# JiLiBIT/LIO-SLAM

Hardware: AMD Instinct MI355X
Metric: scan-to-map registrations/sec, 64x1800 scan vs 200-keyframe map; pose RMSE (higher is better)
Workload: dtype f32

## Files before the change

### include/liogpu.h

```cpp
#ifndef LIOGPU_H
#define LIOGPU_H

#include <stddef.h>
#include <stdint.h>

#ifdef __cplusplus
extern "C" {
#endif

#define LIO_VERSION 102
#define LIO_MAX_ITERS 32

enum {
    LIO_OK               = 0,
    LIO_TOO_FEW_POINTS   = 1,
    LIO_TOO_FEW_CORR     = 2,
    LIO_ERR_ARG          = -1,
    LIO_ERR_HIP          = -2,
    LIO_ERR_CAPACITY     = -3,
    LIO_ERR_NO_MAP       = -4,
    LIO_ERR_NO_DEVICE    = -5
};

typedef struct lio_s2m_config {
// ... 109 lines not shown
                                 float *coeff4, int32_t *nn_idx5);

int  lio_s2m_set_corner_map(lio_s2m_handle *h, const void *pts, size_t n, size_t stride_bytes);
int  lio_s2m_batch_upload_corners(lio_s2m_handle *h, int32_t n_scans, const void *const *scans,
                                  const size_t *n_pts, size_t stride_bytes);
int  lio_s2m_register_cs(lio_s2m_handle *h, const void *corner_scan, size_t n_corner,
                         const void *surf_scan, size_t n_surf, size_t stride_bytes,
                         float pose[6], lio_s2m_result *res);
int  lio_s2m_get_corner_correspondences(lio_s2m_handle *h, int32_t scan, uint8_t *flag,
                                        float *coeff4, int32_t *nn_idx5);

int  lio_s2m_get_profile(lio_s2m_handle *h, lio_s2m_profile *out);
int  lio_s2m_debug_persist_spin(lio_s2m_handle *h, int32_t spin_max, int32_t withhold_wg);

int  lio_debug_plane_fit(int32_t device_id, const float *sets, size_t n, double plane_tol, uint32_t *out);
int  lio_s2m_debug_stamps(lio_s2m_handle *h, long long *out, size_t cap_entries);

int  lio_s2m_set_stream(lio_s2m_handle *h, void *hip_stream);
int  lio_s2m_set_global_grid(lio_s2m_handle *h, const float origin[3], const int32_t dims[3]);
int  lio_s2m_set_shard(lio_s2m_handle *h, int32_t axis, int32_t lo, int32_t hi);
int  lio_s2m_set_shard_plan(lio_s2m_handle *h, int32_t axis, int32_t n_ranks, int32_t rank, const int32_t *bounds,
                            int32_t halo_cells);
int  lio_s2m_set_scan_shard(lio_s2m_handle *h, int32_t rank, int32_t world);
int  lio_s2m_batch_begin(lio_s2m_handle *h);
int  lio_s2m_batch_iter_partial(lio_s2m_handle *h, double *d_sums );
int  lio_s2m_batch_iter_apply(lio_s2m_handle *h, const double *d_sums);
int  lio_s2m_batch_n_active(lio_s2m_handle *h, int32_t *n_active);
int  lio_s2m_batch_poll_active(lio_s2m_handle *h, int32_t iteration, int32_t *n_active);

void lio_transform_update(float pose[6], int32_t imu_available, int32_t imu_type,
// ... 311 lines not shown
```

### lio-slam_amd/__init__.py

```python
from .api import (LioError, ScanToMap, S2MConfig, S2MResult, S2MProfile, DeskewConfig,
                  lib_path, load_library, build_library, deskew, curvature, imu_deskew_info,
                  transform_update, pack_xyzirt, deskew_default_config, voxel_grid, assemble_map, KeyframeStore, STATUS_NAMES,
                  extract_features, FeatureConfig, range_image, RangeImageConfig, PinnedBuffer, DeviceBuffer, PC2Layout, deskew_pc2,
                  NearbyConfig, nearby_default_config, IcpConfig, IcpResult, IcpClouds, ICP_STATES, icp_default_config, icp_align,
                  icp_debug_trace, ScConfig, ScResult, sc_default_config, sc_make, sc_distance,
                  LocalMapConfig, LocalMapInfo, sor_filter, local_map_default_config,
                  HeightMapConfig, HeightMapInfo, height_map, height_map_default_config,
                  GlobalMapConfig, GlobalMapInfo, ExportConfig, global_map_default_config, STAGED_DS, STAGED_RAW)

__all__ = ["LioError", "ScanToMap", "S2MConfig", "S2MResult", "S2MProfile", "DeskewConfig",
           "lib_path", "load_library", "build_library", "deskew", "curvature", "imu_deskew_info",
           "transform_update", "pack_xyzirt", "deskew_default_config", "voxel_grid", "assemble_map", "KeyframeStore", "STATUS_NAMES",
           "extract_features", "FeatureConfig", "range_image", "RangeImageConfig", "PinnedBuffer", "DeviceBuffer", "PC2Layout", "deskew_pc2",
           "NearbyConfig", "nearby_default_config", "IcpConfig", "IcpResult", "IcpClouds", "ICP_STATES", "icp_default_config", "icp_align",
           "icp_debug_trace", "ScConfig", "ScResult", "sc_default_config", "sc_make", "sc_distance",
           "LocalMapConfig", "LocalMapInfo", "sor_filter", "local_map_default_config",
           "HeightMapConfig", "HeightMapInfo", "height_map", "height_map_default_config",
           "GlobalMapConfig", "GlobalMapInfo", "ExportConfig", "global_map_default_config", "STAGED_DS", "STAGED_RAW"]
```

### lio-slam_amd/api.py

```python
import ctypes as C
import os
import subprocess

import numpy as np

_HERE = os.path.dirname(os.path.abspath(__file__))
LIO_MAX_ITERS = 32
STATUS_NAMES = {0: "OK", 1: "TOO_FEW_POINTS", 2: "TOO_FEW_CORR", -1: "ERR_ARG", -2: "ERR_HIP",
                -3: "ERR_CAPACITY", -4: "ERR_NO_MAP", -5: "ERR_NO_DEVICE"}


class LioError(RuntimeError):
    pass


class S2MConfig(C.Structure):
    _fields_ = [
        ("k", C.c_int32), ("max_sq_dist", C.c_float),
        ("plane_tol", C.c_double), ("weight", C.c_double), ("min_s", C.c_double),
        ("min_corr", C.c_int32), ("max_iters", C.c_int32), ("eig_thresh", C.c_float),
        ("conv_deg", C.c_double), ("conv_cm", C.c_double),
        ("min_scan_pts", C.c_int32), ("jacobian_mode", C.c_int32), ("force_all_iters", C.c_int32),
        ("device_id", C.c_int32), ("cell_size", C.c_float), ("max_batch", C.c_int32),
        ("max_scan_pts", C.c_int32), ("record_corr_iter", C.c_int32), ("kernel_variant", C.c_int32),
# ... 166 lines not shown
    "lio_curvature", "lio_s2m_debug_stamps", "lio_s2m_batch_poll_active", "lio_voxel_grid", "lio_assemble_map", "lio_kf_store_create", "lio_kf_store_destroy", "lio_kf_store_add",
    "lio_kf_store_count", "lio_kf_store_points", "lio_assemble_map_resident", "lio_s2m_set_scan_shard",
    "lio_s2m_set_corner_map", "lio_s2m_batch_upload_corners", "lio_s2m_register_cs",
    "lio_s2m_get_corner_correspondences", "lio_feature_default_config", "lio_extract_features",
    "lio_range_image_default_config", "lio_range_image",
    "lio_s2m_share_map", "lio_s2m_batch_upload_async", "lio_host_alloc", "lio_host_free", "lio_host_register",
    "lio_host_unregister", "lio_s2m_set_shard_plan", "lio_s2m_register_pc2", "lio_deskew_pc2", "lio_kf_store_add_device", "lio_kf_store_add_from_handle",
    "lio_s2m_register_raw", "lio_s2m_debug_persist_spin", "lio_device_alloc", "lio_device_free", "lio_device_upload",
    "lio_nearby_default_config", "lio_kf_store_set_poses", "lio_assemble_map_nearby", "lio_debug_plane_fit",
    "lio_icp_default_config", "lio_icp_align", "lio_kf_store_loop_icp", "lio_kf_store_detect_loop", "lio_icp_debug_trace",
    "lio_sc_default_config", "lio_sc_make", "lio_sc_distance", "lio_kf_store_sc_add", "lio_kf_store_sc_add_device",
    "lio_kf_store_sc_add_from_handle", "lio_kf_store_sc_count", "lio_kf_store_sc_geometry", "lio_kf_store_sc_get", "lio_kf_store_sc_detect",
    "lio_sor_filter", "lio_local_map_default_config", "lio_kf_store_local_map",
    "lio_height_map_default_config", "lio_height_map", "lio_kf_store_height_map",
    "lio_global_map_default_config", "lio_kf_store_global_map", "lio_kf_store_export_map", "lio_kf_store_get_keyframe",
    "lio_s2m_registered_cloud",
]


def load_library():
    global _LIB
    if _LIB is not None:
        return _LIB
    p = lib_path()
    if not os.path.exists(p):
        raise LioError(f"{p} is missing: run __graft_entry__.build() (hipcc --offload-arch=gfx950). "
                       "There is no CPU fallback.")
    L = C.CDLL(p)
    vp, i32, f32, f64, sz = C.c_void_p, C.c_int32, C.c_float, C.c_double, C.c_size_t
    L.lio_version.restype = C.c_int
    L.lio_last_error.restype = C.c_char_p
# ... 481 lines not shown
    for k, v in kw.items():
        setattr(c, k, v)
    return c


def curvature(rng, device_id=0):
    r = np.ascontiguousarray(rng, np.float32)
    curv = np.zeros(len(r), np.float32)
    picked = np.full(len(r), -1, np.int32)
    label = np.full(len(r), -1, np.int32)
    _check(load_library().lio_curvature(device_id, r.ctypes.data, len(r), curv.ctypes.data,
                                        picked.ctypes.data, label.ctypes.data), "lio_curvature")
    return curv, picked, label


def debug_plane_fit(sets, plane_tol=0.2, device_id=0):
    a = np.ascontiguousarray(sets, np.float32).reshape(-1, 15)
    out = np.zeros((len(a), 8), np.uint32)
    fn = load_library().lio_debug_plane_fit
    fn.argtypes = [C.c_int32, C.c_void_p, C.c_size_t, C.c_double, C.c_void_p]
    _check(fn(device_id, a.ctypes.data, len(a), float(plane_tol), out.ctypes.data), "lio_debug_plane_fit")
    return out


def range_image(records, t_cur, imu, device_id=0, **cfg_overrides):
    L = load_library()
    cfg = RangeImageConfig()
    L.lio_range_image_default_config(C.byref(cfg))
    cfg.device_id = device_id
    for k, v in cfg_overrides.items():
# ... 453 lines not shown
```

### lio-slam_amd/csrc/lio_device_math.h

```cpp
#pragma once
#include <hip/hip_runtime.h>
#include <float.h>
#include <stdint.h>

#define LIO_DEV __device__ __forceinline__

#ifndef LIO_SHARED_DIV
#define LIO_SHARED_DIV 1
#endif
struct LioDivisor { float d, r; bool mid; };

LIO_DEV bool lio_div_mid(float lo, float hi) { return lo >= 0x1p-40f && hi < 0x1p40f; }

LIO_DEV LioDivisor lio_divisor(float d)
{
    LioDivisor v;
    const float r0 = __builtin_amdgcn_rcpf(d);
    const float e = __builtin_fmaf(-d, r0, 1.0f);
    v.d = d; v.r = __builtin_fmaf(e, r0, r0);
    v.mid = lio_div_mid(fabsf(d), fabsf(d));
    return v;
}

LIO_DEV float lio_div_fast(float n, const LioDivisor& v)
// ... 147 lines not shown
            if (c[i] != 0.0f) {
                c[i] /= a[i][i];
#pragma unroll
                for (int r = 0; r < i; ++r) c[r] -= c[i] * a[r][i];
            }
        }
    }
    const float v0 = (0 < nz) ? c[0] : 0.0f;
    const float v1 = (1 < nz) ? c[1] : 0.0f;
    const float v2 = (2 < nz) ? c[2] : 0.0f;
#pragma unroll
    for (int j = 0; j < 3; ++j)
        x[j] = (p0 == j) ? v0 : (p1 == j) ? v1 : (p2 == j) ? v2 : 0.0f;
}

LIO_DEV bool lio_plane_fit5(const float m[5][3], double plane_tol, float X0[3], float& pa, float& pb, float& pc, float& pd)
{
    float a[5][3];
#pragma unroll
    for (int j = 0; j < 5; ++j) { a[j][0] = m[j][0]; a[j][1] = m[j][1]; a[j][2] = m[j][2]; }
    lio_plane_qr5x3(a, X0);
    pa = X0[0]; pb = X0[1]; pc = X0[2]; pd = 1;
    const float ps = sqrtf(pa * pa + pb * pb + pc * pc);
    const LioDivisor dv = lio_divisor(ps);
    if (LIO_SHARED_DIV && dv.mid && lio_div_mid(lio_min3_abs(pa, pb, pc), lio_max3_abs(pa, pb, pc))) {
        pa = lio_div_fast(pa, dv); pb = lio_div_fast(pb, dv); pc = lio_div_fast(pc, dv); pd = lio_div_fast(pd, dv);
    } else {
        pa /= ps; pb /= ps; pc /= ps; pd /= ps;
    }
    bool planeValid = true;
#pragma unroll
    for (int j = 0; j < 5; ++j) {
        const float v = fabsf(pa * m[j][0] + pb * m[j][1] + pc * m[j][2] + pd);
        if ((double)v > plane_tol) planeValid = false;
    }
    return planeValid;
}

LIO_DEV void lio_jacobian_row(const float tr[6], float px, float py, float pz,
                              float cx, float cy, float cz, float cw, int jac_exact,
                              float row[6], float &rhs)
{
    const float srx = tr[0], crx = tr[1], sry = tr[2], cry = tr[3], srz = tr[4], crz = tr[5];
    const float arx = (-srx * cry * px - (srx * sry * srz + crx * crz) * py + (crx * srz - srx * sry * crz) * pz) * cx
                    + (crx * cry * px - (srx * crz - crx * sry * srz) * py + (crx * sry * crz + srx * srz) * pz) * cy;
    const float mid = jac_exact ? (srx * cry * srz * py) : (srx * sry * srz * py);
    const float ary = (-crx * sry * px + crx * cry * srz * py + crx * cry * crz * pz) * cx
                    + (-srx * sry * px + mid + srx * cry * crz * pz) * cy
                    + (-cry * px - sry * srz * py - sry * crz * pz) * cz;
    const float arz = ((crx * sry * crz + srx * srz) * py + (srx * crz - crx * sry * srz) * pz) * cx
                    + ((-crx * srz + srx * sry * crz) * py + (-srx * sry * srz - crx * crz) * pz) * cy
                    + (cry * crz * py - cry * srz * pz) * cz;
    row[0] = arz; row[1] = ary; row[2] = arx;
    row[3] = cx;  row[4] = cy;  row[5] = cz;
    rhs = -cw;
}

__device__ static float lio_cv_hypot(float a, float b)
{
    a = fabsf(a); b = fabsf(b);
    if (a > b) { b /= a; return a * sqrtf(1 + b * b); }
    if (b > 0) { a /= b; return b * sqrtf(1 + a * a); }
    return 0.0f;
}

LIO_DEV void lio_eigen3_sym(float a00, float a01, float a02, float a11, float a12, float a22,
                            float& e0, float& e1, float axis[3])
// ... 41 lines not shown
#undef LIO_ROT
    }
    int m = 0;
    if (w0 < w1) m = 1;
    if ((m == 0 ? w0 : w1) < w2) m = 2;
    float t0;
#define LIO_SWAP(x, y) do { t0 = (x); (x) = (y); (y) = t0; } while (0)
    if (m == 1) { LIO_SWAP(w0, w1); LIO_SWAP(v00, v10); LIO_SWAP(v01, v11); LIO_SWAP(v02, v12); }
    if (m == 2) { LIO_SWAP(w0, w2); LIO_SWAP(v00, v20); LIO_SWAP(v01, v21); LIO_SWAP(v02, v22); }
    if (w1 < w2) LIO_SWAP(w1, w2);
#undef LIO_SWAP
    e0 = w0; e1 = w1;
    axis[0] = v00; axis[1] = v01; axis[2] = v02;
}

LIO_DEV bool lio_corner_assoc(const float m[5][3], float x0, float y0, float z0, double weight, double min_s,
                              float& ox, float& oy, float& oz, float& ow)
{
    float cx = 0, cy = 0, cz = 0;
#pragma unroll
    for (int j = 0; j < 5; ++j) { cx += m[j][0]; cy += m[j][1]; cz += m[j][2]; }
    cx /= 5; cy /= 5; cz /= 5;
    float a11 = 0, a12 = 0, a13 = 0, a22 = 0, a23 = 0, a33 = 0;
#pragma unroll
    for (int j = 0; j < 5; ++j) {
        const float ax = m[j][0] - cx, ay = m[j][1] - cy, az = m[j][2] - cz;
        a11 += ax * ax; a12 += ax * ay; a13 += ax * az;
        a22 += ay * ay; a23 += ay * az;
        a33 += az * az;
    }
    a11 /= 5; a12 /= 5; a13 /= 5; a22 /= 5; a23 /= 5; a33 /= 5;
// ... 4 lines not shown
    const float x1 = (float)((double)cx + 0.1 * (double)v[0]), y1 = (float)((double)cy + 0.1 * (double)v[1]),
                z1 = (float)((double)cz + 0.1 * (double)v[2]);
    const float x2 = (float)((double)cx - 0.1 * (double)v[0]), y2 = (float)((double)cy - 0.1 * (double)v[1]),
                z2 = (float)((double)cz - 0.1 * (double)v[2]);
    const float m1 = (x0 - x1) * (y0 - y2) - (x0 - x2) * (y0 - y1);
    const float m2 = (x0 - x1) * (z0 - z2) - (x0 - x2) * (z0 - z1);
    const float m3 = (y0 - y1) * (z0 - z2) - (y0 - y2) * (z0 - z1);
    const float a012 = sqrtf(m1 * m1 + m2 * m2 + m3 * m3);
    const float l12 = sqrtf((x1 - x2) * (x1 - x2) + (y1 - y2) * (y1 - y2) + (z1 - z2) * (z1 - z2));
    const float la = ((y1 - y2) * m1 + (z1 - z2) * m2) / a012 / l12;
    const float lb = -((x1 - x2) * m1 - (z1 - z2) * m3) / a012 / l12;
    const float lc = -((x1 - x2) * m2 + (y1 - y2) * m3) / a012 / l12;
    const float ld2 = a012 / l12;
    const float s = (float)(1 - weight * (double)fabsf(ld2));
    ox = s * la; oy = s * lb; oz = s * lc; ow = s * ld2;
    return (double)s > min_s;
}

struct LioSolveWs {
    float A[36];
    float B[36];
    float V2[36];
    float AtA[36];
    float X[6], X2[6];
};

__device__ static __forceinline__ int lio_solve6_qr_reg(float (&A)[36], float (&b)[6])
{
    const float eps = FLT_EPSILON * 10;
    float vl[6], hf[6];
#pragma unroll
// ... 254 lines not shown
```

### lio-slam_amd/csrc/lio_kernels.h

```cpp
#pragma once
#include <hip/hip_runtime.h>
#include "lio_types.h"

struct LioIterParams {
    LioGrid grid;
    LioShard shard;
    LioConsts c;
    const float4* map_sorted;
    const float4* map_xyz4;
    const int* cell_start;
    const float4* nbr_pts;
    const int* nbr_start;
    const float* sx;
    const float* sy;
    const float* sz;
    const int* perm;
    LioScanState* state;
    const LioBlockDesc* blocks;
    double* partials;
    unsigned* arrive;
    int max_blk;
    int xcd_remap;
    int* n_active;
    double* sums_out;
// ... 27 lines not shown
                           int n_blocks, unsigned char* skip, hipStream_t s);
void lio_launch_block_boxes(const LioBlockDesc* blocks, int n_blocks, const LioScanState* st, const float* sx, const float* sy,
                            const float* sz, float* box, hipStream_t s);
void lio_launch_scan_sort_lds(const void* stage, size_t stride, const LioScanState* st, int n_scans, int max_pts, float tile0,
                              int shard_axis, int* perm, float* x, float* y, float* z, hipStream_t s);
void lio_launch_scan_bbox(const void* stage, size_t stride, const LioBlockDesc* prep_blocks, int n_prep_blocks,
                          const LioScanState* st, unsigned* bbox, hipStream_t s);
void lio_launch_scan_tile_sort(const void* stage, size_t stride, int total_pts,
                               const LioBlockDesc* prep_blocks, int n_prep_blocks,
                               const LioScanState* st, const LioScanTiles* tiles, int n_keys,
                               int* key_of, int* key_count, int* key_start, int* tile_sums,
                               int* tmp_idx, int* perm, int* big_list, int* big_cnt,
                               float* x, float* y, float* z, hipStream_t s);
void lio_launch_exclusive_scan(const int* in, int n, int* tile_sums, int* out, hipStream_t s);
void lio_launch_xyzi4_to_soa(const float4* src, int n, float* x, float* y, float* z, float4* xyz4, hipStream_t s);
void lio_launch_debug_plane_fit(const float* sets, long long n, double plane_tol, unsigned* out, hipStream_t s);
```

### lio-slam_amd/csrc/lio_kernels.hip

```cpp
#include <hip/hip_runtime.h>
#include "lio_types.h"
#include "lio_device_math.h"
#include "lio_kernels.h"

#include "lio_s2m_device.h"
#include "lio_scan2.h"
#include "lio_wg.h"

__global__ void k_aos_to_soa(const unsigned char* __restrict__ src, size_t stride, int n,
                             float* __restrict__ x, float* __restrict__ y, float* __restrict__ z,
                             float4* __restrict__ xyz4 )
{
    int i = blockIdx.x * blockDim.x + threadIdx.x;
    if (i >= n) return;
    const float* p = reinterpret_cast<const float*>(src + (size_t)i * stride);
    const float a = p[0], b = p[1], c = p[2];
    x[i] = a; y[i] = b; z[i] = c;
    if (xyz4) xyz4[i] = make_float4(a, b, c, 0.0f);
}

__global__ void k_xyzi4_to_soa(const float4* __restrict__ src, int n, float* __restrict__ x, float* __restrict__ y,
                               float* __restrict__ z, float4* __restrict__ xyz4)
{
    const int i = blockIdx.x * blockDim.x + threadIdx.x;
// ... 550 lines not shown

template <bool SINGLE>
__global__ void k_s2m_init_state(LioScanState* __restrict__ st, int n_scans,
                                 float* __restrict__ poses, int from_state, LioConsts c, int* __restrict__ n_active)
{
    const int s = blockIdx.x * blockDim.x + threadIdx.x;
    bool enough = false;
    if (s < n_scans) {
        LioScanState* p = &st[s];
        float T[12], trig[6], pose[6];
        if (from_state) { for (int k = 0; k < 6; ++k) { pose[k] = p->pose[k]; poses[s * 6 + k] = pose[k]; } }
        else { for (int k = 0; k < 6; ++k) { pose[k] = poses[s * 6 + k]; p->pose[k] = pose[k]; } }
        lio_pose_to_transform(pose, T, trig);
        for (int k = 0; k < 12; ++k) p->T[k] = T[k];
        for (int k = 0; k < 6; ++k) p->trig[k] = trig[k];
        p->iter = 0; p->converged = 0; p->n_corr_last = 0;
        for (int k = 0; k < 32; ++k) { p->n_corr_iter[k] = 0; for (int j = 0; j < 6; ++j) p->pose_iter[k][j] = 0.0f; }
        for (int k = 0; k < 36; ++k) p->AtA[k] = 0.0f;
        for (int k = 0; k < 6; ++k) p->AtB[k] = 0.0f;
        enough = p->n_pts > c.min_scan_pts;
        p->done = enough ? 0 : 1;
        p->status = enough ? 0 : 1;
    }
    if (SINGLE) {
        const int n = __syncthreads_count(enough ? 1 : 0);
        if (threadIdx.x == 0) *n_active = n;
    } else if (enough) {
        atomicAdd(n_active, 1);
    }
}
// ... 229 lines not shown

        if (P.d5_cache && inr[pp])
            P.d5_cache[ci] = ok ? d2_5 : -1.0f;
        float cxx = 0.0f, cyy = 0.0f, czz = 0.0f, cww = 0.0f;
        bool accept = false;
        if (ok) accept = lio_assoc_point<CORNER>(P, nn, qx[pp], qy[pp], qz[pp], px[pp], py[pp], pz[pp], cxx, cyy, czz, cww);
        if (record && inr[pp]) {
            const int li = bd.first + pp * LIO_BLOCK + (int)threadIdx.x;
            const int oi = P.perm ? P.perm[base + li] : base + li;
            P.rec_flag[oi] = accept ? 1 : 0;
            reinterpret_cast<float4*>(P.rec_coeff)[oi] = make_float4(cxx, cyy, czz, cww);
#pragma unroll
            for (int j = 0; j < 5; ++j) P.rec_nn[(size_t)oi * 5 + j] = ok ? nn[j] : -1;
        }
        float row[6] = { 0.0f, 0.0f, 0.0f, 0.0f, 0.0f, 0.0f }, rhs = 0.0f;
        if (accept) lio_jacobian_row(tr, px[pp], py[pp], pz[pp], cxx, cyy, czz, cww, P.c.jac_exact, row, rhs);
        if (PPT > 1) __syncthreads();
        {
            double2* dst = reinterpret_cast<double2*>(s_rows[threadIdx.x]);
            dst[0] = make_double2((double)row[0], (double)row[1]);
            dst[1] = make_double2((double)row[2], (double)row[3]);
            dst[2] = make_double2((double)row[4], (double)row[5]);
            dst[3] = make_double2((double)rhs, accept ? 1.0 : 0.0);
        }
        if (pp == 0) LIO_STAMP(3);
        __syncthreads();
        if (red_s < 28) {
#pragma unroll 8
            for (int p = red_g; p < LIO_BLOCK; p += 8)
                red_acc = __builtin_fma(s_rows[p][red_a], s_rows[p][red_b], red_acc);
        }
// ... 4 lines not shown
    LIO_STAMP(5);
    if (wave != 0) return;

    double* part = P.partials + ((size_t)bd.scan * P.max_blk + bd.blk) * LIO_SUMS;
    if (lane < 28) {
        double v = s_part[0][lane];
#pragma unroll
        for (int w = 1; w < 8; ++w) v += s_part[w][lane];
        __hip_atomic_store(part + lane, v, __ATOMIC_RELAXED, __HIP_MEMORY_SCOPE_AGENT);
    }
    lio_arrive_and_finish(P, bd, st, lane, s_sum, &s_ws, stamp);
    LIO_STAMP(7);
#undef LIO_STAMP
}

__global__ __launch_bounds__(256) void k_debug_plane_fit(const float* __restrict__ sets, long long n, double plane_tol,
                                                         unsigned* __restrict__ out)
{
    const long long i = (long long)blockIdx.x * 256 + threadIdx.x;
    if (i >= n) return;
    float m[5][3];
#pragma unroll
    for (int j = 0; j < 5; ++j)
#pragma unroll
        for (int c = 0; c < 3; ++c) m[j][c] = sets[i * 15 + j * 3 + c];
    float X0[3], pa, pb, pc, pd;
    const bool valid = lio_plane_fit5(m, plane_tol, X0, pa, pb, pc, pd);
    uint4* o = reinterpret_cast<uint4*>(out + i * 8);
    o[0] = make_uint4(__float_as_uint(X0[0]), __float_as_uint(X0[1]), __float_as_uint(X0[2]), __float_as_uint(pa));
    o[1] = make_uint4(__float_as_uint(pb), __float_as_uint(pc), __float_as_uint(pd), valid ? 1u : 0u);
}

void lio_launch_debug_plane_fit(const float* sets, long long n, double plane_tol, unsigned* out, hipStream_t s)
{
    if (n <= 0) return;
    hipLaunchKernelGGL(k_debug_plane_fit, dim3((unsigned)((n + 255) / 256)), dim3(256), 0, s, sets, n, plane_tol, out);
}

__global__ void k_s2m_pack_summary(const LioScanState* __restrict__ st, int n_scans, float* __restrict__ out)
{
    const int s = blockIdx.x * blockDim.x + threadIdx.x;
    if (s >= n_scans) return;
    float* o = out + (size_t)s * 10;
    for (int k = 0; k < 6; ++k) o[k] = st[s].pose[k];
    o[6] = __int_as_float(st[s].iter); o[7] = __int_as_float(st[s].status | (st[s].done ? 0 : 0x100));
    o[8] = __int_as_float(st[s].converged); o[9] = __int_as_float(st[s].is_degenerate);
}

__global__ void k_s2m_apply(LioScanState* __restrict__ st, int n_scans, const double* __restrict__ sums, size_t slot_stride, int n_slots,
                            LioConsts c, int* __restrict__ n_active)
{
// ... 224 lines not shown
```

### lio-slam_amd/csrc/lio_persist.hip

```cpp
#include <hip/hip_runtime.h>
#ifndef LIO_PREFETCH
#define LIO_PREFETCH 2
#endif
#include "lio_kernels.h"
#include "lio_device_math.h"
#include "lio_s2m_device.h"

namespace {

__global__ __launch_bounds__(LIO_BLOCK, 2) void k_s2m_persist(LioIterParams P, unsigned* __restrict__ gen, unsigned epoch, const unsigned char* __restrict__ stage, unsigned stride,
                   int n_main, unsigned* __restrict__ spec, double* __restrict__ spec_sums, const float* __restrict__ poses0,
                   unsigned spin_max, int withhold_wg)
{
    __shared__ __attribute__((aligned(16))) double s_rows[LIO_BLOCK][8];
    __shared__ double s_part[8][28];
    __shared__ double s_sum[28];
    __shared__ LioSolveWs s_ws;
    __shared__ int s_ctl;

    const int wg = blockIdx.x;
    if (wg >= n_main) {
        const int scan = wg - n_main;
        if (threadIdx.x >= 64) return;
        const int hl = threadIdx.x;
// ... 113 lines not shown
        const int nn[5] = { lio_key_idx(top.k0), lio_key_idx(top.k1), lio_key_idx(top.k2), lio_key_idx(top.k3), lio_key_idx(top.k4) };
        if (P.d5_cache && inr) P.d5_cache[ci] = ok ? lio_key_d2(top.k4) : -1.0f;
        LIO_TICK(1);

        float cxx = 0.0f, cyy = 0.0f, czz = 0.0f, cww = 0.0f;
        bool accept = false;
        if (ok) accept = lio_assoc_point<false>(P, nn, qx, qy, qz, px, py, pz, cxx, cyy, czz, cww);
        if (record && inr) {
            const int oi = P.perm ? P.perm[base + li] : base + li;
            P.rec_flag[oi] = accept ? 1 : 0;
            reinterpret_cast<float4*>(P.rec_coeff)[oi] = make_float4(cxx, cyy, czz, cww);
#pragma unroll
            for (int j = 0; j < 5; ++j) P.rec_nn[(size_t)oi * 5 + j] = ok ? nn[j] : -1;
        }
        float row[6] = { 0.0f, 0.0f, 0.0f, 0.0f, 0.0f, 0.0f }, rhs = 0.0f;
        if (accept) lio_jacobian_row(tr, px, py, pz, cxx, cyy, czz, cww, P.c.jac_exact, row, rhs);
        {
            double2* dst = reinterpret_cast<double2*>(s_rows[threadIdx.x]);
            dst[0] = make_double2((double)row[0], (double)row[1]);
            dst[1] = make_double2((double)row[2], (double)row[3]);
            dst[2] = make_double2((double)row[4], (double)row[5]);
            dst[3] = make_double2((double)rhs, accept ? 1.0 : 0.0);
        }
        __syncthreads();
        LIO_TICK(2);
        double red_acc = 0.0;
        if (red_s < 28) {
#pragma unroll 8
            for (int p = red_g; p < LIO_BLOCK; p += 8)
                red_acc = __builtin_fma(s_rows[p][red_a], s_rows[p][red_b], red_acc);
            s_part[red_g][red_s] = red_acc;
// ... 125 lines not shown
```

### lio-slam_amd/csrc/lio_s2m_device.h

```cpp
#pragma once
#include <hip/hip_runtime.h>
#include "lio_types.h"
#include "lio_device_math.h"
#include "lio_kernels.h"

#define LIO_MAX_COORD 1.0e15f
#ifndef LIO_PREFETCH
#define LIO_PREFETCH 1
#endif
#ifndef LIO_ARRIVE_ACQREL
#define LIO_ARRIVE_ACQREL 0
#endif
#define LIO_IDX_MASK 0x1fffffff

LIO_DEV int lio_cell_coord(float v, float origin, float inv_cell, int n)
{
    float c = floorf((v - origin) * inv_cell);
    c = fminf(fmaxf(c, -4.0f), (float)(n + 3));
    return (int)c;
}

LIO_DEV double lio_dmin(double a, double b) { double r; asm("v_min_f64 %0, %1, %2" : "=v"(r) : "v"(a), "v"(b)); return r; }
LIO_DEV double lio_dmax(double a, double b) { double r; asm("v_max_f64 %0, %1, %2" : "=v"(r) : "v"(a), "v"(b)); return r; }

// ... 137 lines not shown
        st->done = done;
        st->status = (nc < c.min_corr) ? 2 : 0;
        if (done && n_active) atomicSub(n_active, 1);
    }
    done = __shfl(done, 0);
    if (!done) {
        float Tn[12], trn[6];
        lio_pose_to_transform_wave(pose, Tn, trn, lane);
        if (lane == 0) {
#pragma unroll
            for (int k = 0; k < 12; ++k) st->Tp[k] = st->T[k];
#pragma unroll
            for (int k = 0; k < 12; ++k) st->T[k] = Tn[k];
#pragma unroll
            for (int k = 0; k < 6; ++k) st->trig[k] = trn[k];
        }
    }
    return 0;
}

typedef float lio_f2 __attribute__((ext_vector_type(2)));

LIO_DEV void lio_knn_pair(const float4& a, const float4& b, lio_f2 qx, lio_f2 qy, lio_f2 qz, double& k0, double& k1)
{
    const lio_f2 X = { a.x, a.y }, Y = { a.z, a.w }, Z = { b.x, b.y };
    const lio_f2 dx = X - qx, dy = Y - qy, dz = Z - qz;
    const lio_f2 d2 = (dx * dx + dy * dy) + dz * dz;
    k0 = lio_make_key(d2.x, __float_as_int(b.z));
    k1 = lio_make_key(d2.y, __float_as_int(b.w));
}
// ... 109 lines not shown
    }
}

template <bool CORNER>
LIO_DEV bool lio_assoc_point(const LioIterParams& P, const int nn[5], float qx, float qy, float qz,
                             float px, float py, float pz, float& cxx, float& cyy, float& czz, float& cww)
{
    bool accept = false;
    float m[5][3];
#pragma unroll
    for (int j = 0; j < 5; ++j) {
        const float4 mp = P.map_xyz4[nn[j]];
        m[j][0] = mp.x; m[j][1] = mp.y; m[j][2] = mp.z;
    }
    if (CORNER) {
        accept = lio_corner_assoc(m, qx, qy, qz, P.c.weight, P.c.min_s, cxx, cyy, czz, cww);
    } else {
        float X0[3], pa, pb, pc, pd;
        const bool planeValid = lio_plane_fit5(m, P.c.plane_tol, X0, pa, pb, pc, pd);
        if (planeValid) {
            const float pd2 = pa * qx + pb * qy + pc * qz + pd;
            const float r2 = px * px + py * py + pz * pz;
            const float s = (float)(1 - P.c.weight * (double)fabsf(pd2) / (double)sqrtf(sqrtf(r2)));
            cxx = s * pa; cyy = s * pb; czz = s * pc; cww = s * pd2;
            accept = (double)s > P.c.min_s;
        }
    }
    return accept;
}

static __constant__ int c_pair_a[32] = { 0,0,0,0,0,0, 1,1,1,1,1, 2,2,2,2, 3,3,3, 4,4, 5,  0,1,2,3,4,5, 7, 0,0,0,0 };
static __constant__ int c_pair_b[32] = { 0,1,2,3,4,5, 1,2,3,4,5, 2,3,4,5, 3,4,5, 4,5, 5,  6,6,6,6,6,6, 7, 0,0,0,0 };

LIO_DEV void lio_arrive_and_finish(const LioIterParams& P, const LioBlockDesc& bd, LioScanState* st, int lane,
                                   double* s_sum, LioSolveWs* s_ws, long long* stamp)
{
#if !LIO_ARRIVE_ACQREL
    asm volatile("s_waitcnt vmcnt(0)" ::: "memory");
#endif
    int last = 0;
    if (lane == 0) {
#if LIO_ARRIVE_ACQREL
        const unsigned old = __hip_atomic_fetch_add(&P.arrive[bd.scan], 1u, __ATOMIC_ACQ_REL, __HIP_MEMORY_SCOPE_AGENT);
// ... 30 lines not shown
```

### lio-slam_amd/csrc/lio_types.h

```cpp
#pragma once
#include <stdint.h>

#define LIO_SUMS 32
#define LIO_SUM_NC 27
#define LIO_BLOCK 256
#define LIO_ROW_ALIGN 8

#define LIO_TB_MAX 3
struct LioGrid {
    float ox, oy, oz;
    float inv_cell;
    int32_t nx, ny, nz;
    int32_t n_cells;
    int32_t k;
    int32_t xs;
    int32_t nxf;
    float inv_cell_x;
    int32_t tb_row0[LIO_TB_MAX], tb_ny[LIO_TB_MAX], tb_nz[LIO_TB_MAX];
    float tb_oy[LIO_TB_MAX], tb_oz[LIO_TB_MAX], tb_inv_cell[LIO_TB_MAX], tb_reach[LIO_TB_MAX];
    int32_t tb_try;
    float tb_try_b2[LIO_TB_MAX];
};

struct LioShard {
    float gorigin;
    float inv_cell;
    int32_t axis;
    int32_t gdim;
    int32_t lo, hi;
};

struct LioConsts {
    double plane_tol, weight, min_s, conv_deg, conv_cm;
    float  max_sq_dist, eig_thresh;
    float  gate_reach;
    int32_t min_corr, max_iters, jac_exact, force_all, record_iter, min_scan_pts;
};

struct LioScanState {
    float pose[6];
    float T[12];
    float Tp[12];
    float trig[6];
    int32_t n_pts;
    int32_t offset;
    int32_t c_n_pts;
    int32_t c_offset;
    int32_t iter;
    int32_t done;
    int32_t converged;
    int32_t is_degenerate;
    int32_t n_corr_last;
    int32_t status;
    float matP[36];
    float AtA[36];
    float AtB[6];
    int32_t n_corr_iter[32];
    float pose_iter[32][6];
// ... 17 lines not shown
```

### lio-slam_amd/csrc/liogpu_api.hip

```cpp
#include <hip/hip_runtime.h>
#include <math.h>
#include <stdio.h>
#include <string.h>
#include <algorithm>
#include <chrono>
#include <exception>
#include <memory>
#include <mutex>
#include <vector>

#include "lio_handle.h"
#include "lio_multi.h"
#include "lio_wg.h"


static thread_local char g_last_error[512];

int lio_fail(int code, const char* what, hipError_t e)
{
    if (e != hipSuccess) snprintf(g_last_error, sizeof(g_last_error), "%s: %s", what, hipGetErrorString(e));
    else snprintf(g_last_error, sizeof(g_last_error), "%s", what);
    return code;
}

// ... 41 lines not shown
    c->cell_div = 2;
    c->xcd_remap = 1;
    c->tile_size = 0.0f;
    c->use_graph = 0;
    c->sort_batch = 1;
    c->graph_iters = 4;
    c->sort_scan = 1;
    c->nn_cache = 1;
    c->pipeline = 0;
    c->n_devices = 1;
    for (int i = 0; i < 8; ++i) c->device_ids[i] = i;
    c->x_sub = 0;
    c->tight_rows = 0;
}

static void lio_fill_consts(lio_s2m_handle* h)
{
    const lio_s2m_config& g = h->cfg;
    h->c.plane_tol = g.plane_tol; h->c.weight = g.weight; h->c.min_s = g.min_s;
    h->c.conv_deg = g.conv_deg; h->c.conv_cm = g.conv_cm;
    h->c.max_sq_dist = g.max_sq_dist; h->c.eig_thresh = g.eig_thresh;
    {
        volatile float r = sqrtf(g.max_sq_dist);
        r = r * 1.0001f;
        r = r + 1e-6f;
        h->c.gate_reach = r;
    }
    h->c.min_corr = g.min_corr; h->c.max_iters = g.max_iters;
    h->c.jac_exact = g.jacobian_mode ? 1 : 0; h->c.force_all = g.force_all_iters ? 1 : 0;
    h->c.record_iter = g.record_corr_iter; h->c.min_scan_pts = g.min_scan_pts;
}

static int lio_s2m_init_resources(lio_s2m_handle* h)
{
    HIPCHK(hipStreamCreateWithFlags(&h->stream, hipStreamNonBlocking));
    for (int i = 0; i < LIO_MAX_ITERS; ++i) {
// ... 439 lines not shown
    h->persist_withhold = withhold_wg;
    return LIO_OK;
} LIO_CATCH

extern "C" int lio_debug_plane_fit(int32_t device_id, const float* sets, size_t n, double plane_tol, uint32_t* out)
try {
    if ((!sets || !out) && n) return lio_fail(LIO_ERR_ARG, "null pointer");
    if (n > ((size_t)1 << 27)) return lio_fail(LIO_ERR_CAPACITY, "at most 2^27 sets per call");
    if (!n) return LIO_OK;
    HIPCHK(hipSetDevice(device_id));
    LioDevBuf<float> d_sets;
    LioDevBuf<unsigned> d_out;
    HIPCHK(d_sets.grow(n * 15, 1.0, 0));
    HIPCHK(d_out.grow(n * 8, 1.0, 0));
    HIPCHK(hipMemcpy(d_sets, sets, n * 15 * sizeof(float), hipMemcpyHostToDevice));
    lio_launch_debug_plane_fit(d_sets, (long long)n, plane_tol, d_out, nullptr);
    HIPCHK(hipGetLastError());
    HIPCHK(hipMemcpy(out, d_out, n * 8 * sizeof(unsigned), hipMemcpyDeviceToHost));
    return LIO_OK;
} LIO_CATCH

static int lio_ensure_soa(lio_s2m_handle* h)
{
    if (h->soa_valid || !h->total_pts) return LIO_OK;
    lio_launch_aos_to_soa(h->last_stage + h->last_xyz_off, h->last_stride, (int)h->total_pts, h->d_sx, h->d_sy, h->d_sz, nullptr, h->stream);
    h->soa_valid = true;
    HIPCHK(hipGetLastError());
    return LIO_OK;
}

extern "C" int lio_s2m_batch_upload(lio_s2m_handle* h, int32_t n_scans, const void* const* scans,
                                    const size_t* n_pts, size_t stride)
try {
// ... 1025 lines not shown
```

Baseline: 436,200.

## Precompute per-scan Jacobian trig coefficients and compare thresholds in float

Per-pose trigonometric product coefficients for the Jacobian row are computed once per pose update and stored in the scan state. Per-point kernels then read them (via constant address space in one path) instead of recomputing the products. Plane-validity and min_s thresholds are also converted once on the host to the largest float not above the double value, which removes double-precision compares in the inner loop. In exchange the scan state grows and each point loads 20 floats, and a debug kernel is added to check the tabulated rows against the original formula.

```diff
diff --git a/include/liogpu.h b/include/liogpu.h
--- a/include/liogpu.h
+++ b/include/liogpu.h
@@ -147,6 +147,10 @@
 int  lio_s2m_debug_persist_spin(lio_s2m_handle *h, int32_t spin_max, int32_t withhold_wg);
 
 int  lio_debug_plane_fit(int32_t device_id, const float *sets, size_t n, double plane_tol, uint32_t *out);
+
+int  lio_debug_jacobian_row(int32_t device_id, const float *in, const int32_t *jac_exact, size_t n, uint32_t *out);
+
+float lio_float_below(double t);
 int  lio_s2m_debug_stamps(lio_s2m_handle *h, long long *out, size_t cap_entries);
 
 int  lio_s2m_set_stream(lio_s2m_handle *h, void *hip_stream);
diff --git a/lio-slam_amd/__init__.py b/lio-slam_amd/__init__.py
--- a/lio-slam_amd/__init__.py
+++ b/lio-slam_amd/__init__.py
@@ -6,7 +6,8 @@
                   icp_debug_trace, ScConfig, ScResult, sc_default_config, sc_make, sc_distance,
                   LocalMapConfig, LocalMapInfo, sor_filter, local_map_default_config,
                   HeightMapConfig, HeightMapInfo, height_map, height_map_default_config,
-                  GlobalMapConfig, GlobalMapInfo, ExportConfig, global_map_default_config, STAGED_DS, STAGED_RAW)
+                  GlobalMapConfig, GlobalMapInfo, ExportConfig, global_map_default_config, STAGED_DS, STAGED_RAW,
+                  debug_jacobian_row, float_below)
 
 __all__ = ["LioError", "ScanToMap", "S2MConfig", "S2MResult", "S2MProfile", "DeskewConfig",
            "lib_path", "load_library", "build_library", "deskew", "curvature", "imu_deskew_info",
@@ -16,4 +17,5 @@
            "icp_debug_trace", "ScConfig", "ScResult", "sc_default_config", "sc_make", "sc_distance",
            "LocalMapConfig", "LocalMapInfo", "sor_filter", "local_map_default_config",
            "HeightMapConfig", "HeightMapInfo", "height_map", "height_map_default_config",
-           "GlobalMapConfig", "GlobalMapInfo", "ExportConfig", "global_map_default_config", "STAGED_DS", "STAGED_RAW"]
+           "GlobalMapConfig", "GlobalMapInfo", "ExportConfig", "global_map_default_config", "STAGED_DS", "STAGED_RAW",
+           "debug_jacobian_row", "float_below"]
diff --git a/lio-slam_amd/api.py b/lio-slam_amd/api.py
--- a/lio-slam_amd/api.py
+++ b/lio-slam_amd/api.py
@@ -204,7 +204,7 @@
     "lio_sor_filter", "lio_local_map_default_config", "lio_kf_store_local_map",
     "lio_height_map_default_config", "lio_height_map", "lio_kf_store_height_map",
     "lio_global_map_default_config", "lio_kf_store_global_map", "lio_kf_store_export_map", "lio_kf_store_get_keyframe",
-    "lio_s2m_registered_cloud",
+    "lio_s2m_registered_cloud", "lio_debug_jacobian_row", "lio_float_below",
 ]
 
 
@@ -716,6 +716,24 @@
     return curv, picked, label
 
 
+def debug_jacobian_row(inputs, jac_exact, device_id=0):
+    a = np.ascontiguousarray(inputs, np.float32).reshape(-1, 13)
+    ex = np.ascontiguousarray(jac_exact, np.int32).reshape(-1)
+    assert len(ex) == len(a)
+    out = np.zeros((len(a), 2, 7), np.uint32)
+    fn = load_library().lio_debug_jacobian_row
+    fn.argtypes = [C.c_int32, C.c_void_p, C.c_void_p, C.c_size_t, C.c_void_p]
+    _check(fn(device_id, a.ctypes.data, ex.ctypes.data, len(a), out.ctypes.data), "lio_debug_jacobian_row")
+    return out
+
+
+def float_below(t):
+    fn = load_library().lio_float_below
+    fn.argtypes = [C.c_double]
+    fn.restype = C.c_float
+    return np.float32(fn(float(t)))
+
+
 def debug_plane_fit(sets, plane_tol=0.2, device_id=0):
     a = np.ascontiguousarray(sets, np.float32).reshape(-1, 15)
     out = np.zeros((len(a), 8), np.uint32)
diff --git a/lio-slam_amd/csrc/lio_device_math.h b/lio-slam_amd/csrc/lio_device_math.h
--- a/lio-slam_amd/csrc/lio_device_math.h
+++ b/lio-slam_amd/csrc/lio_device_math.h
@@ -2,6 +2,7 @@
 #include <hip/hip_runtime.h>
 #include <float.h>
 #include <stdint.h>
+#include "lio_types.h"
 
 #define LIO_DEV __device__ __forceinline__
 
@@ -185,7 +186,7 @@
         x[j] = (p0 == j) ? v0 : (p1 == j) ? v1 : (p2 == j) ? v2 : 0.0f;
 }
 
-LIO_DEV bool lio_plane_fit5(const float m[5][3], double plane_tol, float X0[3], float& pa, float& pb, float& pc, float& pd)
+LIO_DEV bool lio_plane_fit5(const float m[5][3], float plane_tol_f, float X0[3], float& pa, float& pb, float& pc, float& pd)
 {
     float a[5][3];
 #pragma unroll
@@ -203,14 +204,17 @@
 #pragma unroll
     for (int j = 0; j < 5; ++j) {
         const float v = fabsf(pa * m[j][0] + pb * m[j][1] + pc * m[j][2] + pd);
-        if ((double)v > plane_tol) planeValid = false;
+        if (v > plane_tol_f) planeValid = false;
     }
     return planeValid;
 }
 
-LIO_DEV void lio_jacobian_row(const float tr[6], float px, float py, float pz,
-                              float cx, float cy, float cz, float cw, int jac_exact,
-                              float row[6], float &rhs)
+#ifndef LIO_JAC_TABLE
+#define LIO_JAC_TABLE 1
+#endif
+LIO_DEV void lio_jacobian_row_plain(const float tr[6], float px, float py, float pz,
+                                    float cx, float cy, float cz, float cw, int jac_exact,
+                                    float row[6], float &rhs)
 {
     const float srx = tr[0], crx = tr[1], sry = tr[2], cry = tr[3], srz = tr[4], crz = tr[5];
     const float arx = (-srx * cry * px - (srx * sry * srz + crx * crz) * py + (crx * srz - srx * sry * crz) * pz) * cx
@@ -222,6 +226,49 @@
     const float arz = ((crx * sry * crz + srx * srz) * py + (srx * crz - crx * sry * srz) * pz) * cx
                     + ((-crx * srz + srx * sry * crz) * py + (-srx * sry * srz - crx * crz) * pz) * cy
                     + (cry * crz * py - cry * srz * pz) * cz;
+    row[0] = arz; row[1] = ary; row[2] = arx;
+    row[3] = cx;  row[4] = cy;  row[5] = cz;
+    rhs = -cw;
+}
+
+LIO_DEV void lio_jacobian_coeffs(const float tr[6], int jac_exact, float jac[LIO_JAC_N])
+{
+    const float srx = tr[0], crx = tr[1], sry = tr[2], cry = tr[3], srz = tr[4], crz = tr[5];
+    jac[0]  = -srx * cry;
+    jac[1]  = srx * sry * srz + crx * crz;
+    jac[2]  = crx * srz - srx * sry * crz;
+    jac[3]  = crx * cry;
+    jac[4]  = srx * crz - crx * sry * srz;
+    jac[5]  = crx * sry * crz + srx * srz;
+    jac[6]  = jac_exact ? (srx * cry * srz) : (srx * sry * srz);
+    jac[7]  = -crx * sry;
+    jac[8]  = crx * cry * srz;
+    jac[9]  = crx * cry * crz;
+    jac[10] = -srx * sry;
+    jac[11] = srx * cry * crz;
+    jac[12] = -cry;
+    jac[13] = sry * srz;
+    jac[14] = sry * crz;
+    jac[15] = -crx * srz + srx * sry * crz;
+    jac[16] = -srx * sry * srz - crx * crz;
+    jac[17] = cry * crz;
+    jac[18] = cry * srz;
+#pragma unroll
+    for (int k = 19; k < LIO_JAC_N; ++k) jac[k] = 0.0f;
+}
+
+LIO_DEV void lio_jacobian_row_tab(const float jac[LIO_JAC_N], float px, float py, float pz,
+                                  float cx, float cy, float cz, float cw, float row[6], float &rhs)
+{
+    const float arx = (jac[0] * px - jac[1] * py + jac[2] * pz) * cx
+                    + (jac[3] * px - jac[4] * py + jac[5] * pz) * cy;
+    const float mid = jac[6] * py;
+    const float ary = (jac[7] * px + jac[8] * py + jac[9] * pz) * cx
+                    + (jac[10] * px + mid + jac[11] * pz) * cy
+                    + (jac[12] * px - jac[13] * py - jac[14] * pz) * cz;
+    const float arz = (jac[5] * py + jac[4] * pz) * cx
+                    + (jac[15] * py + jac[16] * pz) * cy
+                    + (jac[17] * py - jac[18] * pz) * cz;
     row[0] = arz; row[1] = ary; row[2] = arx;
     row[3] = cx;  row[4] = cy;  row[5] = cz;
     rhs = -cw;
@@ -293,7 +340,7 @@
     axis[0] = v00; axis[1] = v01; axis[2] = v02;
 }
 
-LIO_DEV bool lio_corner_assoc(const float m[5][3], float x0, float y0, float z0, double weight, double min_s,
+LIO_DEV bool lio_corner_assoc(const float m[5][3], float x0, float y0, float z0, double weight, float min_s_f,
                               float& ox, float& oy, float& oz, float& ow)
 {
     float cx = 0, cy = 0, cz = 0;
@@ -328,7 +375,7 @@
     const float ld2 = a012 / l12;
     const float s = (float)(1 - weight * (double)fabsf(ld2));
     ox = s * la; oy = s * lb; oz = s * lc; ow = s * ld2;
-    return (double)s > min_s;
+    return s > min_s_f;
 }
 
 struct LioSolveWs {
diff --git a/lio-slam_amd/csrc/lio_kernels.h b/lio-slam_amd/csrc/lio_kernels.h
--- a/lio-slam_amd/csrc/lio_kernels.h
+++ b/lio-slam_amd/csrc/lio_kernels.h
@@ -65,4 +65,5 @@
                                float* x, float* y, float* z, hipStream_t s);
 void lio_launch_exclusive_scan(const int* in, int n, int* tile_sums, int* out, hipStream_t s);
 void lio_launch_xyzi4_to_soa(const float4* src, int n, float* x, float* y, float* z, float4* xyz4, hipStream_t s);
-void lio_launch_debug_plane_fit(const float* sets, long long n, double plane_tol, unsigned* out, hipStream_t s);
+void lio_launch_debug_plane_fit(const float* sets, long long n, float plane_tol_f, unsigned* out, hipStream_t s);
+void lio_launch_debug_jacobian_row(const float* in, const int* jac_exact, long long n, unsigned* out, hipStream_t s);
diff --git a/lio-slam_amd/csrc/lio_kernels.hip b/lio-slam_amd/csrc/lio_kernels.hip
--- a/lio-slam_amd/csrc/lio_kernels.hip
+++ b/lio-slam_amd/csrc/lio_kernels.hip
@@ -588,6 +588,9 @@
         lio_pose_to_transform(pose, T, trig);
         for (int k = 0; k < 12; ++k) p->T[k] = T[k];
         for (int k = 0; k < 6; ++k) p->trig[k] = trig[k];
+        float jac[LIO_JAC_N];
+        lio_jacobian_coeffs(trig, c.jac_exact, jac);
+        for (int k = 0; k < LIO_JAC_N; ++k) p->jac[k] = jac[k];
         p->iter = 0; p->converged = 0; p->n_corr_last = 0;
         for (int k = 0; k < 32; ++k) { p->n_corr_iter[k] = 0; for (int j = 0; j < 6; ++j) p->pose_iter[k][j] = 0.0f; }
         for (int k = 0; k < 36; ++k) p->AtA[k] = 0.0f;
@@ -847,7 +850,7 @@
             for (int j = 0; j < 5; ++j) P.rec_nn[(size_t)oi * 5 + j] = ok ? nn[j] : -1;
         }
         float row[6] = { 0.0f, 0.0f, 0.0f, 0.0f, 0.0f, 0.0f }, rhs = 0.0f;
-        if (accept) lio_jacobian_row(tr, px[pp], py[pp], pz[pp], cxx, cyy, czz, cww, P.c.jac_exact, row, rhs);
+        if (accept) lio_jacobian_row_scan<true>(st, tr, px[pp], py[pp], pz[pp], cxx, cyy, czz, cww, P.c.jac_exact, row, rhs);
         if (PPT > 1) __syncthreads();
         {
             double2* dst = reinterpret_cast<double2*>(s_rows[threadIdx.x]);
@@ -882,7 +885,7 @@
 #undef LIO_STAMP
 }
 
-__global__ __launch_bounds__(256) void k_debug_plane_fit(const float* __restrict__ sets, long long n, double plane_tol,
+__global__ __launch_bounds__(256) void k_debug_plane_fit(const float* __restrict__ sets, long long n, float plane_tol_f,
                                                          unsigned* __restrict__ out)
 {
     const long long i = (long long)blockIdx.x * 256 + threadIdx.x;
@@ -893,16 +896,41 @@
 #pragma unroll
         for (int c = 0; c < 3; ++c) m[j][c] = sets[i * 15 + j * 3 + c];
     float X0[3], pa, pb, pc, pd;
-    const bool valid = lio_plane_fit5(m, plane_tol, X0, pa, pb, pc, pd);
+    const bool valid = lio_plane_fit5(m, plane_tol_f, X0, pa, pb, pc, pd);
     uint4* o = reinterpret_cast<uint4*>(out + i * 8);
     o[0] = make_uint4(__float_as_uint(X0[0]), __float_as_uint(X0[1]), __float_as_uint(X0[2]), __float_as_uint(pa));
     o[1] = make_uint4(__float_as_uint(pb), __float_as_uint(pc), __float_as_uint(pd), valid ? 1u : 0u);
 }
 
-void lio_launch_debug_plane_fit(const float* sets, long long n, double plane_tol, unsigned* out, hipStream_t s)
+void lio_launch_debug_plane_fit(const float* sets, long long n, float plane_tol_f, unsigned* out, hipStream_t s)
 {
     if (n <= 0) return;
-    hipLaunchKernelGGL(k_debug_plane_fit, dim3((unsigned)((n + 255) / 256)), dim3(256), 0, s, sets, n, plane_tol, out);
+    hipLaunchKernelGGL(k_debug_plane_fit, dim3((unsigned)((n + 255) / 256)), dim3(256), 0, s, sets, n, plane_tol_f, out);
+}
+
+__global__ __launch_bounds__(256) void k_debug_jacobian_row(const float* __restrict__ in, const int* __restrict__ jac_exact, long long n,
+                                                            unsigned* __restrict__ out)
+{
+    const long long i = (long long)blockIdx.x * 256 + threadIdx.x;
+    if (i >= n) return;
+    float v[13];
+#pragma unroll
+    for (int k = 0; k < 13; ++k) v[k] = in[i * 13 + k];
+    const int ex = jac_exact[i];
+    float jac[LIO_JAC_N], row_t[6], rhs_t, row_p[6], rhs_p;
+    lio_jacobian_coeffs(v, ex, jac);
+    lio_jacobian_row_tab(jac, v[6], v[7], v[8], v[9], v[10], v[11], v[12], row_t, rhs_t);
+    lio_jacobian_row_plain(v, v[6], v[7], v[8], v[9], v[10], v[11], v[12], ex, row_p, rhs_p);
+    unsigned* o = out + i * 14;
+#pragma unroll
+    for (int k = 0; k < 6; ++k) { o[k] = __float_as_uint(row_t[k]); o[7 + k] = __float_as_uint(row_p[k]); }
+    o[6] = __float_as_uint(rhs_t); o[13] = __float_as_uint(rhs_p);
+}
+
+void lio_launch_debug_jacobian_row(const float* in, const int* jac_exact, long long n, unsigned* out, hipStream_t s)
+{
+    if (n <= 0) return;
+    hipLaunchKernelGGL(k_debug_jacobian_row, dim3((unsigned)((n + 255) / 256)), dim3(256), 0, s, in, jac_exact, n, out);
 }
 
 __global__ void k_s2m_pack_summary(const LioScanState* __restrict__ st, int n_scans, float* __restrict__ out)
diff --git a/lio-slam_amd/csrc/lio_persist.hip b/lio-slam_amd/csrc/lio_persist.hip
--- a/lio-slam_amd/csrc/lio_persist.hip
+++ b/lio-slam_amd/csrc/lio_persist.hip
@@ -151,7 +151,7 @@
             for (int j = 0; j < 5; ++j) P.rec_nn[(size_t)oi * 5 + j] = ok ? nn[j] : -1;
         }
         float row[6] = { 0.0f, 0.0f, 0.0f, 0.0f, 0.0f, 0.0f }, rhs = 0.0f;
-        if (accept) lio_jacobian_row(tr, px, py, pz, cxx, cyy, czz, cww, P.c.jac_exact, row, rhs);
+        if (accept) lio_jacobian_row_scan<false>(st, tr, px, py, pz, cxx, cyy, czz, cww, P.c.jac_exact, row, rhs);
         {
             double2* dst = reinterpret_cast<double2*>(s_rows[threadIdx.x]);
             dst[0] = make_double2((double)row[0], (double)row[1]);
diff --git a/lio-slam_amd/csrc/lio_s2m_device.h b/lio-slam_amd/csrc/lio_s2m_device.h
--- a/lio-slam_amd/csrc/lio_s2m_device.h
+++ b/lio-slam_amd/csrc/lio_s2m_device.h
@@ -175,6 +175,10 @@
             for (int k = 0; k < 12; ++k) st->T[k] = Tn[k];
 #pragma unroll
             for (int k = 0; k < 6; ++k) st->trig[k] = trn[k];
+            float jac[LIO_JAC_N];
+            lio_jacobian_coeffs(trn, c.jac_exact, jac);
+#pragma unroll
+            for (int k = 0; k < LIO_JAC_N; ++k) st->jac[k] = jac[k];
         }
     }
     return 0;
@@ -314,19 +318,40 @@
         m[j][0] = mp.x; m[j][1] = mp.y; m[j][2] = mp.z;
     }
     if (CORNER) {
-        accept = lio_corner_assoc(m, qx, qy, qz, P.c.weight, P.c.min_s, cxx, cyy, czz, cww);
+        accept = lio_corner_assoc(m, qx, qy, qz, P.c.weight, P.c.min_s_f, cxx, cyy, czz, cww);
     } else {
         float X0[3], pa, pb, pc, pd;
-        const bool planeValid = lio_plane_fit5(m, P.c.plane_tol, X0, pa, pb, pc, pd);
+        const bool planeValid = lio_plane_fit5(m, P.c.plane_tol_f, X0, pa, pb, pc, pd);
         if (planeValid) {
             const float pd2 = pa * qx + pb * qy + pc * qz + pd;
             const float r2 = px * px + py * py + pz * pz;
             const float s = (float)(1 - P.c.weight * (double)fabsf(pd2) / (double)sqrtf(sqrtf(r2)));
             cxx = s * pa; cyy = s * pb; czz = s * pc; cww = s * pd2;
-            accept = (double)s > P.c.min_s;
+            accept = s > P.c.min_s_f;
         }
     }
     return accept;
+}
+
+template <bool CONST_MEM>
+LIO_DEV void lio_jacobian_row_scan(const LioScanState* st, const float tr[6], float px, float py, float pz,
+                                   float cx, float cy, float cz, float cw, int jac_exact, float row[6], float &rhs)
+{
+#if LIO_JAC_TABLE
+    float jac[LIO_JAC_N];
+    if (CONST_MEM) {
+        typedef const float __attribute__((address_space(4))) * lio_cfloat_p;
+        const lio_cfloat_p src = (lio_cfloat_p)(uintptr_t)st->jac;
+#pragma unroll
+        for (int k = 0; k < LIO_JAC_N; ++k) jac[k] = src[k];
+    } else {
+#pragma unroll
+        for (int k = 0; k < LIO_JAC_N; ++k) jac[k] = st->jac[k];
+    }
+    lio_jacobian_row_tab(jac, px, py, pz, cx, cy, cz, cw, row, rhs);
+#else
+    lio_jacobian_row_plain(tr, px, py, pz, cx, cy, cz, cw, jac_exact, row, rhs);
+#endif
 }
 
 static __constant__ int c_pair_a[32] = { 0,0,0,0,0,0, 1,1,1,1,1, 2,2,2,2, 3,3,3, 4,4, 5,  0,1,2,3,4,5, 7, 0,0,0,0 };
diff --git a/lio-slam_amd/csrc/lio_types.h b/lio-slam_amd/csrc/lio_types.h
--- a/lio-slam_amd/csrc/lio_types.h
+++ b/lio-slam_amd/csrc/lio_types.h
@@ -4,6 +4,7 @@
 #define LIO_SUMS 32
 #define LIO_SUM_NC 27
 #define LIO_BLOCK 256
+#define LIO_JAC_N 20
 #define LIO_ROW_ALIGN 8
 
 #define LIO_TB_MAX 3
@@ -33,6 +34,7 @@
 struct LioConsts {
     double plane_tol, weight, min_s, conv_deg, conv_cm;
     float  max_sq_dist, eig_thresh;
+    float  plane_tol_f, min_s_f;
     float  gate_reach;
     int32_t min_corr, max_iters, jac_exact, force_all, record_iter, min_scan_pts;
 };
@@ -42,6 +44,7 @@
     float T[12];
     float Tp[12];
     float trig[6];
+    float jac[LIO_JAC_N];
     int32_t n_pts;
     int32_t offset;
     int32_t c_n_pts;
diff --git a/lio-slam_amd/csrc/liogpu_api.hip b/lio-slam_amd/csrc/liogpu_api.hip
--- a/lio-slam_amd/csrc/liogpu_api.hip
+++ b/lio-slam_amd/csrc/liogpu_api.hip
@@ -1,5 +1,6 @@
 #include <hip/hip_runtime.h>
 #include <math.h>
+#include <float.h>
 #include <stdio.h>
 #include <string.h>
 #include <algorithm>
@@ -79,12 +80,23 @@
     c->tight_rows = 0;
 }
 
+extern "C" float lio_float_below(double t)
+{
+    if (t != t) return (float)t;
+    if (t >= (double)FLT_MAX) return t > DBL_MAX ? INFINITY : FLT_MAX;
+    if (t < -(double)FLT_MAX) return -INFINITY;
+    volatile float f = (float)t;
+    if ((double)f > t) f = nextafterf(f, -INFINITY);
+    return f;
+}
+
 static void lio_fill_consts(lio_s2m_handle* h)
 {
     const lio_s2m_config& g = h->cfg;
     h->c.plane_tol = g.plane_tol; h->c.weight = g.weight; h->c.min_s = g.min_s;
     h->c.conv_deg = g.conv_deg; h->c.conv_cm = g.conv_cm;
     h->c.max_sq_dist = g.max_sq_dist; h->c.eig_thresh = g.eig_thresh;
+    h->c.plane_tol_f = lio_float_below(g.plane_tol); h->c.min_s_f = lio_float_below(g.min_s);
     {
         volatile float r = sqrtf(g.max_sq_dist);
         r = r * 1.0001f;
@@ -554,9 +566,29 @@
     HIPCHK(d_sets.grow(n * 15, 1.0, 0));
     HIPCHK(d_out.grow(n * 8, 1.0, 0));
     HIPCHK(hipMemcpy(d_sets, sets, n * 15 * sizeof(float), hipMemcpyHostToDevice));
-    lio_launch_debug_plane_fit(d_sets, (long long)n, plane_tol, d_out, nullptr);
+    lio_launch_debug_plane_fit(d_sets, (long long)n, lio_float_below(plane_tol), d_out, nullptr);
     HIPCHK(hipGetLastError());
     HIPCHK(hipMemcpy(out, d_out, n * 8 * sizeof(unsigned), hipMemcpyDeviceToHost));
+    return LIO_OK;
+} LIO_CATCH
+
+extern "C" int lio_debug_jacobian_row(int32_t device_id, const float* in, const int32_t* jac_exact, size_t n, uint32_t* out)
+try {
+    if ((!in || !jac_exact || !out) && n) return lio_fail(LIO_ERR_ARG, "null pointer");
+    if (n > ((size_t)1 << 27)) return lio_fail(LIO_ERR_CAPACITY, "at most 2^27 rows per call");
+    if (!n) return LIO_OK;
+    HIPCHK(hipSetDevice(device_id));
+    LioDevBuf<float> d_in;
+    LioDevBuf<int> d_ex;
+    LioDevBuf<unsigned> d_out;
+    HIPCHK(d_in.grow(n * 13, 1.0, 0));
+    HIPCHK(d_ex.grow(n, 1.0, 0));
+    HIPCHK(d_out.grow(n * 14, 1.0, 0));
+    HIPCHK(hipMemcpy(d_in, in, n * 13 * sizeof(float), hipMemcpyHostToDevice));
+    HIPCHK(hipMemcpy(d_ex, jac_exact, n * sizeof(int), hipMemcpyHostToDevice));
+    lio_launch_debug_jacobian_row(d_in, d_ex, (long long)n, d_out, nullptr);
+    HIPCHK(hipGetLastError());
+    HIPCHK(hipMemcpy(out, d_out, n * 14 * sizeof(unsigned), hipMemcpyDeviceToHost));
     return LIO_OK;
 } LIO_CATCH
 
```

Result: faster. 441,700 (median of 6 runs) (+1.3%).
